# solonas13/REAL

Hardware: NVIDIA B200
Metric: matching-path reads/s (higher is better)
Workload: dtype u64

## Files before the change

### real_b200/csrc/index.cuh

```cuda
#pragma once

#include "common.cuh"
#include "prims.cuh"

namespace realgpu
{

__host__ __device__ __forceinline__ int list_of(int table, int t)
{
        return table == 0 ? (t == 0 ? 0 : (t == 1 ? 3 : 5)) : (table == 1 ? (t == 0 ? 1 : 4) : 2);
}
__host__ __device__ __forceinline__ int pair_second(int table, int t) { return t + 1 + table; }

__host__ __device__ __forceinline__ int table_lists(int table, uint32_t seedkmax)
{
        if ( seedkmax >= 2 ) return table == 0 ? 3 : (table == 1 ? 2 : 1);
        if ( seedkmax == 1 ) return table == 0 ? 2 : (table == 1 ? 1 : 0);
        return table == 0 ? 1 : 0;
}


__device__ __forceinline__ uint64_t pack_bytes(const uint8_t * __restrict__ p, uint32_t len, uint32_t & bad)
{
        uintptr_t const addr = reinterpret_cast<uintptr_t>(p);
// ... 661 lines not shown
                #pragma unroll
                for ( int k = 0; k < 4; ++k )
                        if ( i0 + (uint32_t)k * 256 < s1 )
                        {
                                uint32_t const l = entry_slot(seed[k], G, val[k] & 3) - slot0;
                                atomicOr(&bits[l >> 5], 1u << (l & 31));
                        }
        }
        __syncthreads();
        uint32_t const wpt = (words + 255) / 256;
        uint32_t const w0 = threadIdx.x * wpt;
        uint32_t c = 0;
        for ( uint32_t w = w0; w < min(words, w0 + wpt); ++w ) c += __popc(bits[w]);
        uint32_t d;
        uint32_t run = s0 + block_excl_scan(c, &d);
        for ( uint32_t w = w0; w < min(words, w0 + wpt); ++w ) { rank[w] = run; run += __popc(bits[w]); }
        __syncthreads();
        for ( uint32_t w = threadIdx.x; w < words; w += 256 )
        {
                SlotWord sw; sw.bits = bits[w]; sw.rank = rank[w];
                slots[(uint64_t)sb * words + w] = sw;
        }
        for ( uint32_t r = threadIdx.x; r < d; r += 256 ) E[s0 + r].next = ENTRY_NONE;
        if ( threadIdx.x == 0 && d ) atomicAdd(ndistinct, d);
        __syncthreads();
        for ( uint32_t i0 = s0 + threadIdx.x; i0 < s1; i0 += 1024 )
        {
                uint64_t seed[4]; uint32_t val[4];
                #pragma unroll
                for ( int k = 0; k < 4; ++k )
                {
                        uint32_t const i = i0 + (uint32_t)k * 256;
                        seed[k] = (i < s1) ? __ldg(ent_seed + i) : 0;
                        val[k] = (i < s1) ? __ldg(ent_val + i) : 0;
                }
                #pragma unroll
                for ( int k = 0; k < 4; ++k )
                        if ( i0 + (uint32_t)k * 256 < s1 )
                        {
                                uint32_t const l = entry_slot(seed[k], G, val[k] & 3) - slot0;
                                uint32_t const bit = 1u << (l & 31);
                                uint32_t const r = rank[l >> 5] + __popc(bits[l >> 5] & (bit - 1));
                                if ( ! (atomicOr(&claimed[l >> 5], bit) & bit) )
                                {
                                        E[r].seed = seed[k];
                                        E[r].val = val[k];
                                }
                                else
                                {
                                        uint32_t const j = atomicAdd(&ndup, 1u);
                                        if ( j < SUB_DUP_CAP )
                                        {
                                                SubDup dd; dd.seed = seed[k]; dd.val = val[k]; dd.r = r;
                                                dup[j] = dd;
                                        }
                                        else
                                        {
                                                uint32_t const o = s0 + d + SUB_DUP_CAP + atomicAdd(&ovf, 1u);
                                                Entry en; en.seed = seed[k]; en.val = val[k];
                                                en.next = atomicExch(&E[r].next, o);
                                                E[o] = en;
                                        }
                                }
                        }
        }
        __syncthreads();
        uint32_t const nd = min(ndup, SUB_DUP_CAP);
        for ( uint32_t j = threadIdx.x; j < nd; j += 256 )
        {
                SubDup const dd = dup[j];
                uint32_t const o = s0 + d + j;
                Entry en; en.seed = dd.seed; en.val = dd.val;
                en.next = atomicExch(&E[dd.r].next, o);
                E[o] = en;
        }
}

static const uint32_t SUB3_DUP_CAP = 256;
struct Build3Params
{
        const uint64_t * item_seed; const uint32_t * item_val; const uint32_t * sub_start;
        TableGeom G[3];
        uint32_t sub_shift, words, first_sub;
        SlotWord * slots[3]; Entry * E[3];
        uint32_t * ndistinct[3];
};

template<bool FAST>
__device__ __forceinline__ uint32_t sub_local_slot(uint64_t seed, TableGeom const & G, uint32_t t, int tb, uint32_t slot0)
{
        if ( FAST )
                return (uint32_t)(seed >> (16u * (2u - t - (uint32_t)tb))) & 0xFFFFu;
        return entry_slot(seed, G, t) - slot0;
}

#ifndef REAL_BUILD_MINB
#define REAL_BUILD_MINB 6
#endif
template<bool SPLIT, bool FAST>
__global__ void __launch_bounds__(256, SPLIT ? REAL_BUILD_MINB : 3) k_build_sub3(const __grid_constant__ Build3Params P)
{
        extern __shared__ __align__(16) uint32_t sub_smem[];
        uint32_t const words = P.words;
        constexpr int NT = SPLIT ? 1 : 3;
        __shared__ SubDup dup[NT][SUB3_DUP_CAP];
        __shared__ uint32_t ndup[NT], dist[NT];
        uint32_t const sb = P.first_sub + (SPLIT ? blockIdx.x / 3 : blockIdx.x);
        int const tb0 = SPLIT ? (int)(blockIdx.x % 3) : 0;
        if ( SPLIT && ! P.G[tb0].nlists ) return;
        uint32_t const s0 = P.sub_start[sb], s1 = P.sub_start[sb+1];
        uint32_t const slot0 = sb << P.sub_shift;
        uint32_t const tstride = 2 * words + (words + 1) / 2;
        for ( uint32_t i = s0 + threadIdx.x * 16; i < s1; i += 256 * 16 )
        {
                asm volatile("prefetch.global.L2 [%0];" :: "l"(P.item_seed + i));
                if ( ((i - s0) & 31) == 0 ) asm volatile("prefetch.global.L2 [%0];" :: "l"(P.item_val + i));
        }
        for ( uint32_t w = threadIdx.x; w < NT * tstride; w += 256 ) sub_smem[w] = 0;
        if ( threadIdx.x < NT ) ndup[threadIdx.x] = 0;
        __syncthreads();
        for ( uint32_t i0 = s0 + threadIdx.x; i0 < s1; i0 += 1024 )
        {
                uint64_t seed[4]; uint32_t val[4];
                #pragma unroll
                for ( int k = 0; k < 4; ++k )
                {
                        uint32_t const i = i0 + (uint32_t)k * 256;
                        seed[k] = (i < s1) ? __ldg(P.item_seed + i) : 0;
                        val[k] = (i < s1) ? __ldg(P.item_val + i) : 0;
                }
                #pragma unroll
                for ( int k = 0; k < 4; ++k )
                        if ( i0 + (uint32_t)k * 256 < s1 )
                        {
                                uint32_t const t = val[k] & 3;
                                #pragma unroll
                                for ( int u = 0; u < NT; ++u )
                                {
                                        int const tb = tb0 + u;
                                        if ( t < P.G[tb].nlists )
                                        {
                                                uint32_t const l = sub_local_slot<FAST>(seed[k], P.G[tb], t, tb, slot0);
                                                atomicOr(&sub_smem[u * tstride + (l >> 5)], 1u << (l & 31));
                                        }
                                }
                        }
        }
        __syncthreads();
        uint32_t const wpt = (words + 255) / 256;
        uint32_t const w0 = threadIdx.x * wpt;
        #pragma unroll 1
        for ( int u = 0; u < NT; ++u )
        {
                uint32_t * bits = sub_smem + u * tstride;
                uint16_t * rank = reinterpret_cast<uint16_t *>(bits + 2 * words);
                uint32_t c = 0;
                for ( uint32_t w = w0; w < min(words, w0 + wpt); ++w ) c += __popc(bits[w]);
                uint32_t d;
                uint32_t run = block_excl_scan(c, &d);
                for ( uint32_t w = w0; w < min(words, w0 + wpt); ++w ) { rank[w] = (uint16_t)run; run += __popc(bits[w]); }
                if ( threadIdx.x == 0 ) dist[u] = d;
        }
        __syncthreads();
        #pragma unroll 1
        for ( int u = 0; u < NT; ++u )
        {
// ... 2 lines not shown
                const uint32_t * bits = sub_smem + u * tstride;
                const uint16_t * rank = reinterpret_cast<const uint16_t *>(bits + 2 * words);
                for ( uint32_t w = threadIdx.x; w < words; w += 256 )
                {
                        SlotWord sw; sw.bits = bits[w]; sw.rank = s0 + rank[w];
                        P.slots[tb][(uint64_t)sb * words + w] = sw;
                }
                if ( threadIdx.x == 0 && dist[u] ) atomicAdd(P.ndistinct[tb], dist[u]);
        }
        __syncthreads();
        for ( uint32_t i0 = s0 + threadIdx.x; i0 < s1; i0 += 1024 )
        {
                uint64_t seed[4]; uint32_t val[4];
                #pragma unroll
                for ( int k = 0; k < 4; ++k )
                {
                        uint32_t const i = i0 + (uint32_t)k * 256;
                        seed[k] = (i < s1) ? __ldg(P.item_seed + i) : 0;
                        val[k] = (i < s1) ? __ldg(P.item_val + i) : 0;
                }
                #pragma unroll
                for ( int k = 0; k < 4; ++k )
                        if ( i0 + (uint32_t)k * 256 < s1 )
                        {
                                uint32_t const t = val[k] & 3;
                                #pragma unroll
                                for ( int u = 0; u < NT; ++u )
                                {
                                        int const tb = tb0 + u;
                                        if ( t < P.G[tb].nlists )
                                        {
                                                uint32_t * bits = sub_smem + u * tstride, * claimed = bits + words;
                                                const uint16_t * rank = reinterpret_cast<const uint16_t *>(bits + 2 * words);
                                                uint32_t const l = sub_local_slot<FAST>(seed[k], P.G[tb], t, tb, slot0);
                                                uint32_t const bit = 1u << (l & 31);
                                                uint32_t const r = s0 + rank[l >> 5] + __popc(bits[l >> 5] & (bit - 1));
                                                Entry * E = P.E[tb];
                                                if ( ! (atomicOr(&claimed[l >> 5], bit) & bit) )
                                                {
                                                        Entry en; en.seed = seed[k]; en.val = val[k]; en.next = ENTRY_NONE;
                                                        *reinterpret_cast<uint4 *>(E + r) = *reinterpret_cast<const uint4 *>(&en);
                                                }
                                                else
                                                {
                                                        uint32_t const j = atomicAdd(&ndup[u], 1u);
                                                        if ( j < SUB3_DUP_CAP )
                                                        {
                                                                SubDup dd; dd.seed = seed[k]; dd.val = val[k]; dd.r = r;
                                                                dup[u][j] = dd;
                                                        }
                                                        else
                                                        {
                                                                Entry en; en.seed = seed[k]; en.val = val[k]; en.next = r;
                                                                *reinterpret_cast<uint4 *>(E + s0 + dist[u] + j) = *reinterpret_cast<const uint4 *>(&en);
                                                        }
                                                }
                                        }
                                }
                        }
        }
        __syncthreads();
        #pragma unroll 1
        for ( int u = 0; u < NT; ++u )
        {
                uint32_t const nd = min(ndup[u], SUB3_DUP_CAP);
                Entry * E = P.E[tb0 + u];
                for ( uint32_t j = threadIdx.x; j < nd; j += 256 )
                {
                        SubDup const dd = dup[u][j];
                        uint32_t const o = s0 + dist[u] + j;
                        Entry en; en.seed = dd.seed; en.val = dd.val;
                        en.next = atomicExch(&E[dd.r].next, o);
                        *reinterpret_cast<uint4 *>(E + o) = *reinterpret_cast<const uint4 *>(&en);
                }
                for ( uint32_t j = SUB3_DUP_CAP + threadIdx.x; j < ndup[u]; j += 256 )
                {
                        uint32_t const o = s0 + dist[u] + j;
                        uint32_t const r = E[o].next;
                        E[o].next = atomicExch(&E[r].next, o);
                }
        }
}

}
```

### real_b200/csrc/prims.cuh

```cuda
#pragma once

#include "common.cuh"

namespace realgpu
{


static const int SCAN_THREADS = 256;
static const int SCAN_ITEMS = 8;
static const int SCAN_TILE = SCAN_THREADS * SCAN_ITEMS;

__device__ __forceinline__ uint32_t warp_incl_scan(uint32_t v, int lane)
{
        #pragma unroll
        for ( int o = 1; o < 32; o <<= 1 )
        {
                uint32_t const t = __shfl_up_sync(0xffffffffu, v, o);
                if ( lane >= o ) v += t;
        }
        return v;
}

__device__ __forceinline__ void ballot_bit(uint32_t v, uint32_t mask, uint32_t & bal, uint32_t & flip)
{
        asm volatile("{\n\t"
                     ".reg .pred p;\n\t"
                     ".reg .b32 t;\n\t"
                     "and.b32 t, %2, %3;\n\t"
                     "setp.ne.u32 p, t, 0;\n\t"
                     "vote.sync.ballot.b32 %0, p, 0xffffffff;\n\t"
                     "selp.b32 %1, 0, 0xffffffff, p;\n\t"
                     "}" : "=r"(bal), "=r"(flip) : "r"(v), "r"(mask));
}

__device__ __forceinline__ uint32_t peers_u8(uint32_t v, bool ok)
{
        uint32_t peers = __ballot_sync(0xffffffffu, ok);
        #pragma unroll
        for ( int b = 0; b < 8; ++b )
        {
                uint32_t bal, flip;
                ballot_bit(v, 1u << b, bal, flip);
                peers &= bal ^ flip;
        }
        return peers;
}

__device__ __forceinline__ uint32_t peers_low(uint32_t v, bool ok, uint32_t nbits)
{
        uint32_t peers = __ballot_sync(0xffffffffu, ok);
        #pragma unroll
        for ( int b = 0; b < 8; ++b )
                if ( (uint32_t)b < nbits )
                {
                        uint32_t bal, flip;
                        ballot_bit(v, 1u << b, bal, flip);
                        peers &= bal ^ flip;
                }
        return peers;
}

__device__ __forceinline__ uint32_t block_excl_scan(uint32_t v, uint32_t * total)
{
        __shared__ uint32_t warp_sums[32];
        int const lane = threadIdx.x & 31, wid = threadIdx.x >> 5;
        uint32_t const incl = warp_incl_scan(v, lane);
        if ( lane == 31 ) warp_sums[wid] = incl;
        __syncthreads();
        if ( wid == 0 )
        {
                uint32_t s = (lane < (int)(blockDim.x >> 5)) ? warp_sums[lane] : 0;
                s = warp_incl_scan(s, lane);
                warp_sums[lane] = s;
        }
        __syncthreads();
        uint32_t const base = wid ? warp_sums[wid-1] : 0;
        *total = warp_sums[(blockDim.x >> 5) - 1];
        __syncthreads();
        return base + incl - v;
}

__device__ __forceinline__ uint32_t block_excl_scan256(uint32_t v, uint32_t * total, uint32_t * scratch)
{
        int const lane = threadIdx.x & 31, wid = threadIdx.x >> 5;
        uint32_t const incl = warp_incl_scan(v, lane);
        if ( lane == 31 ) scratch[wid] = incl;
        __syncthreads();
        uint32_t base = 0, all = 0;
        #pragma unroll
        for ( int w = 0; w < 8; ++w )
        {
                uint32_t const x = scratch[w];
                if ( w < wid ) base += x;
// ... 80 lines not shown
```

### real_b200/csrc/real_gpu.cu

```cuda
#include "../../include/real_gpu.h"

#include "common.cuh"
#include "prims.cuh"
#include "index.cuh"
#include "scan.cuh"
#include "post.cuh"
#include "ingest.cuh"
#include "format.cuh"

#include <algorithm>
#include <atomic>
#include <chrono>
#include <thread>
#include <cstring>
#include <cstdlib>
#include <cfloat>
#include <vector>
#include <functional>

using namespace realgpu;

namespace
{

// ... 518 lines not shown
                k_ent_scatter_own<<<(unsigned)std::min<uint64_t>(otiles, (uint64_t)h->sm_count * std::max(1, occ_o)), 256, osmem, h->st>>>(EP);
        }
        else
                k_ent_scatter<<<(unsigned)std::min<uint64_t>(etiles, (uint64_t)h->sm_count * std::max(1, occ)), 256, esmem, h->st>>>(EP);
        RG_KERNEL_CHECK();
        launch_count(h, 2);

        const uint64_t * fin_seed = EP.ent_seed; const uint32_t * fin_val = EP.ent_val; const uint32_t * fin_start = EP.bucket_start;
        if ( TP.e2 )
        {
                RG_CUDA(cudaMemsetAsync(EP.sub_count, 0, (size_t)3 * 65600 * 4, h->st));
                k_ent2_hist<<<(unsigned)(h->sm_count * std::max(1, occh)), 256, 0, h->st>>>(EP);
                RG_KERNEL_CHECK(); launch_count(h);
                uint32_t nl = 0;
                exclusive_scan_u32(EP.sub_count, EP.sub_start, (uint64_t)TP.nsub + 1, ptr<uint32_t>(h->ws_stmp), h->st, &nl);
                launch_count(h, nl);
                k_ent2_scatter<<<(unsigned)(h->sm_count * std::max(1, occ2)), 256, esmem, h->st>>>(EP);
                RG_KERNEL_CHECK(); launch_count(h);
                fin_seed = EP.ent2_seed; fin_val = EP.ent2_val; fin_start = EP.sub_start;
        }
        Grouped G; G.seed = fin_seed; G.val = fin_val; G.start = fin_start;
        return G;
}

void build_table(real_gpu * h, int t, TablePlan const & TP)
{
        if ( TP.empty ) return;
        Table & T = h->tab[t];
        EntryPartParams const & EP = TP.EP;
        Grouped const GR = partition_entries(h, TP);
        const uint64_t * fin_seed = GR.seed; const uint32_t * fin_val = GR.val; const uint32_t * fin_start = GR.start;
        k_build_sub<<<TP.own_subs, 256, (size_t)3 * TP.words * 4, h->st>>>(fin_seed, fin_val, fin_start, EP.G, TP.sub_shift, TP.words, ptr<SlotWord>(T.bitmap), ptr<Entry>(T.E), TP.d_ndist, TP.first_sub);
        RG_KERNEL_CHECK(); launch_count(h);
        RG_CUDA(cudaMemcpyAsync(&h->table_counts[2*t], TP.d_total, 8, cudaMemcpyDeviceToHost, h->st));
}

bool build_tables_fused(real_gpu * h, TablePlan * plan)
{
        uint32_t const hb = h->tab[0].hb, fb = 2 * h->F;
        if ( hb != h->keybits || h->nreads == 0 || plan[0].empty ) return false;
        if ( getenv("REAL_GPU_NO_FUSED_BUILD") ) return false;
        uint32_t const nlA = table_lists(0, h->prm.seedkmax);
        uint64_t const cap_items = h->nreads * 2 * nlA;
        uint32_t const pbmin = hb > 16 ? hb - 16 : 0, pbmax = std::min<uint32_t>(std::min<uint32_t>(16, hb > 5 ? hb - 5 : 0), fb);
        if ( pbmin > pbmax ) return false;
        uint32_t pb = 0;
        while ( (cap_items >> pb) > SUB_TARGET_ENTRIES ) ++pb;
        pb = std::min(std::max(pb, pbmin), pbmax);
        if ( h->comm.nranks > 1 && pb < 8 ) return false;

        TablePlan TP = plan[0];
        uint32_t * meta = TP.EP.bucket_count;
        uint32_t const e1 = std::min<uint32_t>(8, pb);
        TP.e2 = pb - e1; TP.nsub = 1u << pb; TP.sub_shift = hb - pb;
        TP.words = TP.sub_shift >= 5 ? (1u << (TP.sub_shift - 5)) : 1u;
        TP.EP.G.table = TABLE_ITEMS; TP.EP.G.nlists = nlA;
        TP.EP.ebits = e1; TP.EP.e2bits = TP.e2;
        TP.first_sub = 0; TP.own_subs = TP.nsub;
        if ( h->comm.nranks > 1 )
        {
                TP.first_sub = TP.EP.own_lo << (pb - 8);
                TP.own_subs = (TP.EP.own_last + 1 - TP.EP.own_lo) << (pb - 8);
        }
        Build3Params B;
        memset(&B, 0, sizeof(B));
        for ( int t = 0; t < 3; ++t )
        {
                Table & T = h->tab[t];
                T.nblocks = TP.nsub;
                T.bitmap_bytes = (size_t)TP.nsub * TP.words * sizeof(SlotWord);
                dev_reserve(h, T.bitmap, T.bitmap_bytes);
                dev_reserve(h, T.E, std::max<size_t>(16, cap_items * sizeof(Entry)) + 256);
                if ( plan[t].empty ) RG_CUDA(cudaMemsetAsync(T.bitmap.p, 0, T.bitmap_bytes, h->st));
                B.G[t] = plan[t].EP.G; B.G[t].table = t; B.G[t].nlists = plan[t].empty ? 0 : T.nlists;
                B.slots[t] = ptr<SlotWord>(T.bitmap); B.E[t] = ptr<Entry>(T.E);
                B.ndistinct[t] = meta + 521 + t;
        }
        EntryPartParams3 Q;
        for ( int t = 0; t < 3; ++t ) { Q.P[t] = TP.EP; if ( t ) Q.P[t].G.nlists = 0; }
        k_ent_hist3<<<(unsigned)(h->sm_count * 8), 256, 0, h->st>>>(Q);
        RG_KERNEL_CHECK(); launch_count(h);
        Grouped const GR = partition_entries(h, TP);
        B.item_seed = GR.seed; B.item_val = GR.val; B.sub_start = GR.start;
        B.sub_shift = TP.sub_shift; B.words = TP.words; B.first_sub = TP.first_sub;
        bool split = true;
        if ( const char * e = getenv("REAL_GPU_BUILD_SPLIT") ) split = atoi(e) != 0;
        size_t const smem1 = (size_t)(2 * TP.words + (TP.words + 1) / 2) * 4;
        size_t const smem = split ? smem1 : 3 * smem1;
        bool const fast = h->F == 8 && hb == 32 && TP.sub_shift == 16 && ! getenv("REAL_GPU_BUILD_GENERAL");
        typedef void (*build_fn)(const Build3Params);
        build_fn const kb = split ? (fast ? (build_fn)k_build_sub3<true, true> : (build_fn)k_build_sub3<true, false>)
                                  : (fast ? (build_fn)k_build_sub3<false, true> : (build_fn)k_build_sub3<false, false>);
        RG_CUDA(cudaFuncSetAttribute(kb, cudaFuncAttributeMaxDynamicSharedMemorySize, (int)smem));
        kb<<<split ? TP.own_subs * 3 : TP.own_subs, 256, smem, h->st>>>(B);
        RG_KERNEL_CHECK(); launch_count(h);
        RG_CUDA(cudaMemcpyAsync(&h->table_counts[0], TP.d_total, 16, cudaMemcpyDeviceToHost, h->st));
        h->fused_build = true;
        return true;
}

int build_from_device(real_gpu * h)
{
        uint32_t const seedl = std::min<uint32_t>(h->prm.seedl, 32);
        h->F = seedl / 4;
        h->keybits = seedl;
        h->W = std::max<uint32_t>(1, (h->maxlen + 31) / 32);
        uint64_t const nreads = h->nreads;

        RG_CUDA(cudaEventRecord(h->ev[2], h->st));
        if ( ! h->src_packed )
                dev_reserve(h, h->rpack, (size_t)nreads * 2 * h->W * 8 + 16);
        dev_reserve(h, h->rlen, (size_t)nreads * 4 + 16);
        dev_reserve(h, h->seeds, (size_t)nreads * 2 * 8 + 16);
        dev_reserve(h, h->usable, (size_t)nreads * 4 + 16);
        dev_reserve(h, h->bad, (size_t)nreads * 4 + 16);
        if ( ! h->src_packed && h->W > PB_MAX_W )
                RG_CUDA(cudaMemsetAsync(h->bad.p, 0, (size_t)nreads * 4 + 16, h->st));
        if ( nreads )
        {
                if ( ! h->src_packed && h->W <= PB_MAX_W )
                {
                        uint32_t const rpb = 256 / h->W;
                        k_pack_both<<<blocks_for(nreads, rpb), 256, 0, h->st>>>(h->src_mapped, ptr<uint64_t>(h->offs), nreads, h->W, seedl, h->prm.seedl, ptr<uint64_t>(h->rpack),
                                                                                ptr<uint32_t>(h->rlen), ptr<uint64_t>(h->seeds), ptr<uint32_t>(h->usable));
                        RG_KERNEL_CHECK(); launch_count(h);
                }
                else if ( h->src_packed )
                {
                        k_seeds_packed<<<blocks_for(nreads, 256), 256, 0, h->st>>>(h->src_packed, h->src_byte_offsets,
                                                                                 (h->src_packed_uniform || h->src_len32) ? nullptr : ptr<uint64_t>(h->offs), h->src_len32,
                                                                                 h->src_packed_uniform, nreads, seedl, h->prm.seedl, ptr<uint32_t>(h->bad),
                                                                                 ptr<uint32_t>(h->rlen), ptr<uint64_t>(h->seeds), ptr<uint32_t>(h->usable));
                        RG_KERNEL_CHECK(); launch_count(h);
                }
                else
                {
                        k_pack_reads<<<blocks_for(nreads * 2 * h->W, 256), 256, 0, h->st>>>(h->src_mapped, ptr<uint64_t>(h->offs), nreads, h->W,
                                                                                          ptr<uint64_t>(h->rpack), ptr<uint32_t>(h->bad));
                        RG_KERNEL_CHECK(); launch_count(h);
                        k_read_seeds<<<blocks_for(nreads, 256), 256, 0, h->st>>>(ptr<uint64_t>(h->offs), nreads, h->W, seedl, h->prm.seedl, ptr<uint64_t>(h->rpack),
                                                                               ptr<uint32_t>(h->bad), ptr<uint32_t>(h->rlen), ptr<uint64_t>(h->seeds), ptr<uint32_t>(h->usable));
                        RG_KERNEL_CHECK(); launch_count(h);
                }
        }
        RG_CUDA(cudaEventRecord(h->ev[3], h->st));

        uint64_t const maxent = std::max<uint64_t>(1, nreads * 2 * table_lists(0, h->prm.seedkmax));
        uint32_t const hbmax = std::min<uint32_t>(h->keybits, 32);
        dev_reserve(h, h->ws_k0, maxent * 8 + 16);
        dev_reserve(h, h->ws_v0, maxent * 4 + 16);
        dev_reserve(h, h->ws_k1, maxent * 8 + 16);
        dev_reserve(h, h->ws_v1, maxent * 4 + 16);
        dev_reserve(h, h->ws_flags, (size_t)3 * 65600 * 4);
        dev_reserve(h, h->ws_stmp, scan_temp_elems(65600) * 4 + 64);
        dev_reserve(h, h->ws_hist, 3 * TABLE_META_WORDS * 4);
        memset(h->table_counts, 0, 6 * sizeof(uint32_t));
        TablePlan plan[3];
        EntryPartParams3 Q;
        bool any_table = false;
        for ( int t = 0; t < 3; ++t )
        {
                plan[t] = plan_table(h, t, ptr<uint32_t>(h->ws_hist) + (size_t)t * TABLE_META_WORDS);
                Q.P[t] = plan[t].EP;
                any_table = any_table || ! plan[t].empty;
        }
        h->fused_build = false;
        if ( any_table && build_tables_fused(h, plan) )
                any_table = false;
        else
        for ( int t = 0; t < 3 && any_table; ++t )
                if ( ! plan[t].empty )
                {
// ... 458 lines not shown
                        if ( sharded )
                        {
                                comm_signal(h, 0);
                                comm_wait(h, 0, CM.epoch, S.wait_ms);
                                k_comm_pairs<<<1, SC_PAIR_THREADS, 0, h->st>>>(P, reinterpret_cast<uint32_t *>(CM.base[CM.rank] + CM.meta_off));
                                RG_KERNEL_CHECK(); launch_count(h);
                        }
                        mark();
                        if ( h->evp.size() < 2 * (nprobe_ev + 1) )
                        {
                                cudaEvent_t a, b;
                                RG_CUDA(cudaEventCreate(&a)); RG_CUDA(cudaEventCreate(&b));
                                h->evp.push_back(a); h->evp.push_back(b);
                        }
                        if ( h->text_pending ) RG_CUDA(cudaStreamWaitEvent(h->st, h->evc[1], 0));
                        RG_CUDA(cudaEventRecord(h->evp[2 * nprobe_ev], h->st));
                        S.probe<<<(unsigned)(h->sm_count * S.occ_b), SC_THREADS, S.bsmem, h->st>>>(P);
                        RG_KERNEL_CHECK();
                        RG_CUDA(cudaEventRecord(h->evp[2 * nprobe_ev + 1], h->st));
                        ++nprobe_ev;
                        mark();
                        if ( sharded )
                        {
                                comm_signal(h, 1);
                        }
                        launch_count(h);
                        h->stats.scan_launches += 1;
                }
                P.x_begin = x_begin; P.x_end = x_end;
                RG_CUDA(cudaMemcpyAsync(ptr<unsigned long long>(h->counters) + 4, P.nprobed, 8, cudaMemcpyDeviceToDevice, h->st));
                if ( ! sharded && x_end - x_begin <= chunk_cap )
                {
                        R.x_begin = S.x_begin; R.x_end = S.x_end; R.win_begin = P.win_begin; R.win_end = P.win_end; R.chunk_cap = S.chunk_cap;
                        R.bucket_bits = P.bucket_bits; R.own_b_lo = P.own_b_lo; R.own_b_cnt = P.own_b_cnt; R.own_list = S.own_list; R.recs = P.recs;
                        R.valid = true; R.ahead = false;
                }
                if ( trace )
                {
                        RG_CUDA(cudaStreamSynchronize(h->st));
                        static const char * names[6] = { "hist", "wait_consumed", "offsets+scatter", "handover", "probe", "" };
                        for ( size_t i = 0; i + 1 < tev.size(); ++i )
                        {
                                if ( i % 6 == 5 ) continue;
                                fprintf(stderr, "[trace rank %u round %zu] %-16s %8.3f ms\n", CM.rank, i / 6, names[i % 6], elapsed(tev[i], tev[i+1]));
                        }
                        for ( cudaEvent_t e : tev ) cudaEventDestroy(e);
                }
        }
        RG_CUDA(cudaEventRecord(h->ev[6], h->st));
        unsigned long long c[5] = {0, 0, 0, 0, 0};
        RG_CUDA(cudaMemcpyAsync(c, h->counters.p, sizeof(c), cudaMemcpyDeviceToHost, h->st));
        RG_CUDA(cudaStreamSynchronize(h->st));
        R.inflight = false;
        h->stats.scan_ms = elapsed(h->ev[5], h->ev[6]);
        finish_text(h);
        h->stats.probe_ms = 0;
        for ( size_t i = 0; i < nprobe_ev; ++i ) h->stats.probe_ms += elapsed(h->evp[2*i], h->evp[2*i+1]);
        h->stats.part_ms = was_ahead ? elapsed(R.ev0, R.done) : (use_prep ? 0.f : h->stats.scan_ms - h->stats.probe_ms);
        h->stats.prepared_scans += was_ahead ? 1 : 0;
        if ( ! ntiles ) h->stats.n_windows = 0;
        else if ( h->comm.nranks > 1 && ! h->comm.window.p ) h->stats.n_windows = c[4];
        if ( h->comm.nranks > 1 && h->comm.window.p )
        {
                uint32_t cerr = 0;
                RG_CUDA(cudaMemcpy(&cerr, h->comm.error.p, 4, cudaMemcpyDeviceToHost));
                if ( cerr ) throw CudaError("sharded tables: timed out waiting for rank " + std::to_string(cerr - 1));
        }
        uint32_t nt = 0;
        for ( int t = 0; t < 3; ++t ) if ( P.tab[t].nlists ) ++nt;
        h->stats.n_probes = h->stats.n_windows * nt;
        h->stats.n_candidates = c[1];
        h->stats.n_seedpass = c[2];
        h->stats.n_hits = c[3];
        return (mode != 1) ? (uint64_t)c[0] : (uint64_t)c[3];
}

void preload_kernels(int device)
{
        static bool done[64] = { false };
        if ( device < 0 || device >= 64 || done[device] ) return;
        cudaFuncAttributes a;
#define RG_PRELOAD(k) RG_CUDA(cudaFuncGetAttributes(&a, k))
        RG_PRELOAD(k_pack_reads); RG_PRELOAD(k_pack_both); RG_PRELOAD(k_seeds_packed); RG_PRELOAD(k_read_seeds); RG_PRELOAD(k_uniform_offsets); RG_PRELOAD(k_flags_to_bad);
        RG_PRELOAD(k_ent_hist3); RG_PRELOAD(k_ent_offsets); RG_PRELOAD(k_ent_scatter); RG_PRELOAD(k_ent_scatter_own); RG_PRELOAD(k_ent2_hist); RG_PRELOAD(k_ent2_scatter); RG_PRELOAD(k_build_sub); RG_PRELOAD((k_build_sub3<true, true>)); RG_PRELOAD((k_build_sub3<true, false>)); RG_PRELOAD((k_build_sub3<false, true>)); RG_PRELOAD((k_build_sub3<false, false>));
        RG_PRELOAD(k_scan_reduce); RG_PRELOAD(k_scan_apply); RG_PRELOAD(k_fill_f32);
        RG_PRELOAD(k_part_hist); RG_PRELOAD(k_part_offsets); RG_PRELOAD(k_part_scatter<false>); RG_PRELOAD(k_part_scatter<true>); RG_PRELOAD(k_own_list); RG_PRELOAD((k_bucket_probe<false, false>)); RG_PRELOAD((k_bucket_probe<true, false>)); RG_PRELOAD((k_bucket_probe<false, true>)); RG_PRELOAD((k_bucket_probe<true, true>));
        RG_PRELOAD(k_comm_signal); RG_PRELOAD(k_comm_wait); RG_PRELOAD(k_comm_pairs);
        RG_PRELOAD(k_score_hits); RG_PRELOAD(k_hit_count); RG_PRELOAD(k_hit_scatter); RG_PRELOAD(k_hit_order<real_gpu_hit>);
        RG_PRELOAD(k_unique_export); RG_PRELOAD(k_unique_ties); RG_PRELOAD(k_unique_import); RG_PRELOAD(k_unique_replay); RG_PRELOAD(k_fold_push); RG_PRELOAD(k_fold_merge); RG_PRELOAD(k_unique_checksum); RG_PRELOAD(k_mark_large); RG_PRELOAD(k_sort_large<0>); RG_PRELOAD(k_sort_large<1>); RG_PRELOAD(k_sort_large<2>);
        RG_PRELOAD(k_fmt_len<false>); RG_PRELOAD(k_fmt_len<true>); RG_PRELOAD(k_fmt_write<false>); RG_PRELOAD(k_fmt_write<true>);
        RG_PRELOAD(k_fa_summary); RG_PRELOAD(k_rd_table); RG_PRELOAD(k_rd_permute); RG_PRELOAD(k_rd_repack); RG_PRELOAD(k_rd_sums); RG_PRELOAD(k_fa_scan); RG_PRELOAD(k_fa_pack);
        RG_PRELOAD(k_window_counts); RG_PRELOAD(k_block_bounds); RG_PRELOAD(k_gap_dp); RG_PRELOAD(k_gap_replay);
#undef RG_PRELOAD
        done[device] = true;
}

int check_ready(real_gpu * h)
{
        if ( ! h->have_text ) return fail(h, REAL_GPU_E_STATE, "no text set");
        if ( ! h->have_reads ) return fail(h, REAL_GPU_E_STATE, "no reads set");
        if ( std::min<uint64_t>(h->n_total, h->own_end + h->maxlen) > h->shard_begin + h->shard_len )
                return fail(h, REAL_GPU_E_ARG, "the shard does not hold the read-length halo behind its own range (real_gpu_set_text: [own_begin, min(n_total, own_end + maxreadlen)))");
        return REAL_GPU_OK;
}

}


extern "C" {

int real_gpu_abi_version(void) { return REAL_GPU_ABI_VERSION; }

int real_gpu_device_count(void)
{
        int n = 0;
        if ( cudaGetDeviceCount(&n) != cudaSuccess ) { (void)cudaGetLastError(); return 0; }
        return n;
}

int real_gpu_create(const real_gpu_params * params, real_gpu ** out)
{
        if ( ! params || ! out ) return REAL_GPU_E_ARG;
        *out = nullptr;
        if ( params->struct_size != sizeof(real_gpu_params) ) return REAL_GPU_E_ARG;
        real_gpu * h = new real_gpu();
        h->prm = *params;
        h->prm.ll_table = nullptr;
        int code = REAL_GPU_OK;
        try
        {
                if ( params->seedl < 4 || params->seedl > 64 || params->seedl % 4 )
                        throw std::invalid_argument("seed length must be a multiple of 4 in 4..64");
                if ( params->seedkmax > 2 ) throw std::invalid_argument("seedkmax > 2");
                if ( params->totalkmax > 15 ) throw std::invalid_argument("totalkmax > 15");
                if ( params->scores && ! params->ll_table ) throw std::invalid_argument("scores requested without ll_table");
                int ndev = 0;
                RG_CUDA(cudaGetDeviceCount(&ndev));
                if ( params->device < 0 || params->device >= ndev ) throw CudaError("no such CUDA device");
                RG_CUDA(cudaSetDevice(params->device));
                cudaDeviceProp prop;
                RG_CUDA(cudaGetDeviceProperties(&prop, params->device));
                if ( prop.major < 10 ) throw CudaError("device is not sm_100 class; this library only carries sm_100a code");
                h->sm_count = prop.multiProcessorCount;
                preload_kernels(params->device);
                if ( const char * e = getenv("REAL_GPU_PASS_BITS") ) h->pass_bits_override = atoi(e);
                if ( const char * e = getenv("REAL_GPU_L2_SLICE_MB") ) h->l2_slice_bytes = (uint64_t)atoi(e) << 20;
                if ( const char * e = getenv("REAL_GPU_OWN_LIST_MAX") ) h->own_list_max = atoi(e);
                if ( const char * e = getenv("REAL_GPU_AUTO_PREPARE") ) h->auto_prepare = atoi(e) != 0;
                if ( const char * e = getenv("REAL_GPU_CHUNK_MPOS") ) h->chunk_positions = std::max<uint64_t>(SC_TILE_POS, ((uint64_t)atoi(e) << 20) / SC_TILE_POS * SC_TILE_POS);
                RG_CUDA(cudaStreamCreateWithFlags(&h->st, cudaStreamNonBlocking));
                RG_CUDA(cudaStreamCreateWithFlags(&h->st2, cudaStreamNonBlocking));
                RG_CUDA(cudaMallocHost(&h->table_counts, 6 * sizeof(uint32_t)));
                RG_CUDA(cudaMallocHost(&h->fa_totals, 2 * sizeof(uint64_t)));
                for ( int i = 0; i < 8; ++i ) RG_CUDA(cudaEventCreate(&h->ev[i]));
                for ( int i = 0; i < 2; ++i ) RG_CUDA(cudaEventCreate(&h->evc[i]));
                RG_CUDA(cudaEventCreateWithFlags(&h->ev_words, cudaEventDisableTiming));
                if ( params->ll_table )
                {
                        dev_alloc(h, h->ll, 1024 * 8);
                        RG_CUDA(cudaMemcpyAsync(h->ll.p, params->ll_table, 1024 * 8, cudaMemcpyHostToDevice, h->st));
                        RG_CUDA(cudaStreamSynchronize(h->st));
                }
        }
        catch ( std::invalid_argument const & e ) { h->err = e.what(); code = REAL_GPU_E_ARG; }
        catch ( std::exception const & e ) { h->err = e.what(); code = REAL_GPU_E_CUDA; }
        if ( code != REAL_GPU_OK )
        {
// ... 1422 lines not shown
```

### real_b200/csrc/scan.cuh

```cuda
#pragma once

#include "common.cuh"
#include "index.cuh"

namespace realgpu
{

static const int SC_THREADS = 256;
static const int SC_WPT = 2;
static const int SC_TILE_WORDS = SC_THREADS * SC_WPT;
static const int SC_TILE_POS = SC_TILE_WORDS * 32;
static const int SC_HALO = 2;
static const int SC_SMEM_WORDS = SC_TILE_WORDS + 2 * SC_HALO;
static const int SC_MAX_BUCKETS = 256;
static const int SC_CURSOR_STRIDE = 32;
static const int SC_UNIT = 512;
#ifndef REAL_SC_RPT
#define REAL_SC_RPT 2
#endif
#ifndef REAL_PROBE_MINB
#define REAL_PROBE_MINB 3
#endif
static const int SC_RPT = REAL_SC_RPT;
static const int SC_QA_CAP = 32 + 96 * SC_RPT;
static const int SC_QB_CAP = 64;
static const uint32_t SC_POS_NONE = 0xFFFFFFFFu;
static const uint64_t SC_MAX_CHUNK = 0xFFF00000ull;
static const uint64_t SC_MAX_ROUND = 1ull << 30;

static const int SC_MAX_RANKS = 8;
static const int SC_META_STRIDE = SC_MAX_BUCKETS + 8;

struct TableDev
{
        const SlotWord * slots;
        const Entry * E;
        uint32_t hb;
        uint32_t nlists;
};

struct ScanParams
{
        const uint64_t * text;
        const uint64_t * nmask;
        uint64_t shard_begin;
        uint64_t x_begin, x_end;
        uint64_t pos_base;
        uint64_t win_begin, win_end;
        uint64_t own_begin, own_end;
        TableDev tab[3];
        uint32_t seedl, F, keybits, seedkmax, totalkmax;
        uint32_t vseedl;
        ReadSrc rs;
        const uint32_t * rlen;
        const uint64_t * rec;
        uint32_t nrec;
        uint32_t fileid;
        uint32_t bucket_bits;
        uint32_t debug_flags;
        uint4 * recs;
        uint32_t * bucket_count;
        uint32_t * bucket_start;
        uint32_t * bucket_cursor;
        uint32_t * unit_counter;
        int mode;
        RawHit * hits;
        unsigned long long hit_cap;
        unsigned long long * hit_count;
        unsigned long long * info;
        unsigned long long * stats;
        uint32_t nranks, rank;
        uint32_t bucket_lo[SC_MAX_RANKS + 1];
        uint4 * peer_recs[SC_MAX_RANKS];
        uint32_t * peer_meta[SC_MAX_RANKS];
        uint32_t seg_cap;
        uint32_t * pair_grab;
        uint32_t * pair_rec;
        uint32_t npairs;
        uint32_t own_b_lo, own_b_cnt;
        uint32_t hist_pick_max;
        uint32_t * list;
        unsigned long long * list_count;
        unsigned long long * nprobed;
};

__device__ __forceinline__ uint32_t bucket_owner(ScanParams const & P, uint32_t b)
{
        uint32_t r = 0;
        #pragma unroll
        for ( int i = 1; i < SC_MAX_RANKS; ++i )
                if ( (uint32_t)i < P.nranks && b >= P.bucket_lo[i] ) r = i;
        return r;
}

__device__ __forceinline__ uint32_t smem_u32(const void * p) { return (uint32_t)__cvta_generic_to_shared(p); }

__device__ __forceinline__ void mbar_init(uint64_t * bar, uint32_t count)
{
        asm volatile("mbarrier.init.shared::cta.b64 [%0], %1;" :: "r"(smem_u32(bar)), "r"(count));
}
__device__ __forceinline__ void mbar_expect_tx(uint64_t * bar, uint32_t bytes)
{
        asm volatile("mbarrier.arrive.expect_tx.shared::cta.b64 _, [%0], %1;" :: "r"(smem_u32(bar)), "r"(bytes) : "memory");
}
__device__ __forceinline__ void mbar_wait(uint64_t * bar, uint32_t parity)
{
        uint32_t done = 0;
        while ( ! done )
        {
                asm volatile(
                        "{\n\t"
                        ".reg .pred p;\n\t"
                        "mbarrier.try_wait.parity.shared::cta.b64 p, [%1], %2;\n\t"
                        "selp.u32 %0, 1, 0, p;\n\t"
                        "}" : "=r"(done) : "r"(smem_u32(bar)), "r"(parity) : "memory");
        }
}
__device__ __forceinline__ void bulk_load(void * dst, const void * src, uint32_t bytes, uint64_t * bar)
{
        asm volatile("cp.async.bulk.shared::cluster.global.mbarrier::complete_tx::bytes [%0], [%1], %2, [%3];"
                     :: "r"(smem_u32(dst)), "l"(src), "r"(bytes), "r"(smem_u32(bar)) : "memory");
}


__device__ __forceinline__ void unique_update(unsigned long long * slot, uint32_t inverted, uint32_t file, uint64_t pos, uint32_t k, uint32_t frag)
{
        unsigned long long old = *slot;
        while ( true )
        {
                uint32_t const st = umi_state(old);
                unsigned long long const take = umi_make(inverted ? ST_REVERSE : ST_STRAIGHT, file, pos, k, frag);
                unsigned long long neu = old;
                if ( st == ST_NOMATCH || st == ST_GAPPED )
                        neu = take;
                else if ( k < umi_err(old) )
                        neu = take;
                else if ( k == umi_err(old) )
                {
                        bool const same = (pos == umi_pos(old)) && (file == umi_file(old)) && (frag == umi_frag(old));
                        if ( st == ST_NONUNIQUE )
                        {
                                if ( file < umi_file(old) || (file == umi_file(old) && pos < umi_pos(old)) )
                                        neu = umi_with_state(take, ST_NONUNIQUE);
                        }
                        else if ( ! same )
                        {
                                bool const smaller = file < umi_file(old) || (file == umi_file(old) && pos < umi_pos(old));
                                neu = umi_with_state(smaller ? take : old, ST_NONUNIQUE);
                        }
                        else if ( ! inverted && st == ST_REVERSE )
                                neu = take;
                }
                if ( neu == old )
                        return;
                unsigned long long const prev = atomicCAS(slot, old, neu);
                if ( prev == old )
                        return;
                old = prev;
        }
}

__device__ __forceinline__ uint32_t record_of(const uint64_t * __restrict__ rec, uint32_t nrec, uint64_t pos)
{
        uint32_t lo = 0, hi = nrec + 1;
        while ( lo < hi )
        {
                uint32_t const mid = (lo + hi) >> 1;
                if ( __ldg(rec + mid) <= pos ) lo = mid + 1; else hi = mid;
        }
        return lo - 1;
}

__device__ __forceinline__ bool wildcard_free(const uint64_t * __restrict__ nmask, uint64_t lpos, uint32_t len)
{
        uint64_t const first = lpos >> 6, last = (lpos + len - 1) >> 6;
        for ( uint64_t w = first; w <= last; ++w )
        {
                uint64_t m = __ldg(nmask + w);
                if ( m )
                {
                        if ( w == first ) m &= (~0ULL) >> (lpos & 63);
                        if ( w == last ) m &= (~0ULL) << (63 - ((lpos + len - 1) & 63));
                        if ( m ) return false;
                }
        }
        return true;
}



struct HistSmem
{
        uint64_t tile[2][SC_SMEM_WORDS];
        uint64_t bar[2];
        uint32_t cnt[SC_MAX_BUCKETS];
};

__device__ __forceinline__ uint32_t clip_mask(uint64_t lx0, uint64_t x_begin, uint64_t x_end)
{
        if ( lx0 + 32 <= x_begin || lx0 >= x_end ) return 0;
        uint32_t m = 0xFFFFFFFFu;
        if ( lx0 < x_begin ) m &= 0xFFFFFFFFu << (uint32_t)(x_begin - lx0);
        if ( lx0 + 32 > x_end ) m &= 0xFFFFFFFFu >> (uint32_t)(lx0 + 32 - x_end);
        return m;
}

// ... 880 lines not shown
```

Baseline: 579.1 million.

## Add persistent fused 3-table sub-bucket build kernel with bulk-copy double buffering

Adds a persistent kernel that loops over sub-buckets, building all three tables in shared memory per sub-bucket. While one sub-bucket is processed, the next one's seeds and values are prefetched with cp.async.bulk into a second buffer tracked by an mbarrier. The aim is to hide global load latency and avoid per-sub-bucket launch and block scheduling overhead. It uses large shared memory at one block per SM with 1024 threads, which may cut latency hiding elsewhere. Sub-buckets too large for the buffer fall back to reading directly from global memory.

```diff
diff --git a/real_b200/csrc/index.cuh b/real_b200/csrc/index.cuh
--- a/real_b200/csrc/index.cuh
+++ b/real_b200/csrc/index.cuh
@@ -767,6 +767,7 @@
         const uint64_t * item_seed; const uint32_t * item_val; const uint32_t * sub_start;
         TableGeom G[3];
         uint32_t sub_shift, words, first_sub;
+        uint32_t nsubs;
         SlotWord * slots[3]; Entry * E[3];
         uint32_t * ndistinct[3];
 };
@@ -935,4 +936,207 @@
         }
 }
 
-}
+static const uint32_t B3_WORDS = 2048;
+static const uint32_t B3_TSTRIDE = 2 * B3_WORDS + B3_WORDS / 2;
+static const uint32_t B3_ITEM_CAP = 6400;
+template<uint32_t NTHR>
+struct Build3Smem
+{
+        uint64_t seed[2][B3_ITEM_CAP + 2];
+        uint32_t val[2][B3_ITEM_CAP + 8];
+        uint32_t tab[3][B3_TSTRIDE];
+        SubDup dup[3][SUB3_DUP_CAP];
+        uint64_t wsum[NTHR / 32];
+        uint64_t bar[2];
+        uint32_t ndup[3], dist[3];
+};
+
+__device__ __forceinline__ bool b3_fits(uint32_t s0, uint32_t s1) { return s1 > s0 && s1 - s0 <= B3_ITEM_CAP; }
+
+template<uint32_t NTHR>
+__device__ __forceinline__ void b3_fetch(Build3Smem<NTHR> & S, Build3Params const & P, uint32_t buf, uint32_t s0, uint32_t s1)
+{
+        uint32_t const a = s0 & ~1u, b = (s1 + 1) & ~1u, c = s0 & ~3u, d = (s1 + 3) & ~3u;
+        mbar_expect_tx(&S.bar[buf], (b - a) * 8 + (d - c) * 4);
+        bulk_load(S.seed[buf], P.item_seed + a, (b - a) * 8, &S.bar[buf]);
+        bulk_load(S.val[buf], P.item_val + c, (d - c) * 4, &S.bar[buf]);
+}
+
+template<uint32_t NTHR>
+__device__ __forceinline__ void b3_clear(Build3Smem<NTHR> & S)
+{
+        #pragma unroll
+        for ( int tb = 0; tb < 3; ++tb )
+                for ( uint32_t w = threadIdx.x; w < 2 * B3_WORDS / 4; w += NTHR )
+                        reinterpret_cast<uint4 *>(S.tab[tb])[w] = make_uint4(0u, 0u, 0u, 0u);
+}
+
+template<uint32_t NTHR>
+__device__ __forceinline__ void b3_build(Build3Smem<NTHR> & S, Build3Params const & P, uint32_t sb, uint32_t s0, uint32_t n,
+                                         const uint64_t * isd, const uint32_t * ivl)
+{
+        constexpr uint32_t WPT = B3_WORDS / NTHR;
+        static_assert(WPT % 2 == 0, "slot words are stored two at a time");
+        for ( uint32_t i = threadIdx.x; i < n; i += NTHR )
+        {
+                uint64_t const seed = isd[i];
+                uint32_t const t = ivl[i] & 3;
+                #pragma unroll
+                for ( int tb = 0; tb < 3; ++tb )
+                        if ( t < P.G[tb].nlists )
+                        {
+                                uint32_t const l = sub_local_slot<true>(seed, P.G[tb], t, tb, 0);
+                                atomicOr(&S.tab[tb][l >> 5], 1u << (l & 31));
+                        }
+        }
+        __syncthreads();
+        uint32_t const w0 = threadIdx.x * WPT;
+        uint32_t bw[3][WPT];
+        uint64_t cnt = 0;
+        #pragma unroll
+        for ( int tb = 0; tb < 3; ++tb )
+        {
+                uint32_t c = 0;
+                #pragma unroll
+                for ( uint32_t k = 0; k < WPT; ++k ) { bw[tb][k] = S.tab[tb][w0 + k]; c += __popc(bw[tb][k]); }
+                cnt |= (uint64_t)c << (21 * tb);
+        }
+        int const lane = threadIdx.x & 31, wid = threadIdx.x >> 5;
+        uint64_t incl = cnt;
+        #pragma unroll
+        for ( int o = 1; o < 32; o <<= 1 )
+        {
+                uint64_t const x = __shfl_up_sync(0xffffffffu, incl, o);
+                if ( lane >= o ) incl += x;
+        }
+        if ( lane == 31 ) S.wsum[wid] = incl;
+        __syncthreads();
+        uint64_t base = 0, all = 0;
+        #pragma unroll
+        for ( int w = 0; w < (int)(NTHR / 32); ++w )
+        {
+                uint64_t const x = S.wsum[w];
+                if ( w < wid ) base += x;
+                all += x;
+        }
+        uint64_t const ex = base + incl - cnt;
+        #pragma unroll
+        for ( int tb = 0; tb < 3; ++tb )
+        {
+                uint16_t * rank = reinterpret_cast<uint16_t *>(S.tab[tb] + 2 * B3_WORDS);
+                uint32_t run = (uint32_t)(ex >> (21 * tb)) & 0x1FFFFFu;
+                uint32_t rk[WPT];
+                #pragma unroll
+                for ( uint32_t k = 0; k < WPT; ++k ) { rk[k] = run; rank[w0 + k] = (uint16_t)run; run += __popc(bw[tb][k]); }
+                if ( P.G[tb].nlists )
+                {
+                        uint4 * dst = reinterpret_cast<uint4 *>(P.slots[tb] + (uint64_t)sb * B3_WORDS + w0);
+                        #pragma unroll
+                        for ( uint32_t k = 0; k < WPT; k += 2 ) dst[k / 2] = make_uint4(bw[tb][k], s0 + rk[k], bw[tb][k+1], s0 + rk[k+1]);
+                }
+        }
+        if ( threadIdx.x < 3 )
+        {
+                uint32_t const d = (uint32_t)(all >> (21 * threadIdx.x)) & 0x1FFFFFu;
+                S.dist[threadIdx.x] = d;
+                S.ndup[threadIdx.x] = 0;
+                if ( P.G[threadIdx.x].nlists && d ) atomicAdd(P.ndistinct[threadIdx.x], d);
+        }
+        __syncthreads();
+        for ( uint32_t i = threadIdx.x; i < n; i += NTHR )
+        {
+                uint64_t const seed = isd[i];
+                uint32_t const val = ivl[i], t = val & 3;
+                #pragma unroll
+                for ( int tb = 0; tb < 3; ++tb )
+                        if ( t < P.G[tb].nlists )
+                        {
+                                uint32_t * bits = S.tab[tb], * claimed = bits + B3_WORDS;
+                                const uint16_t * rank = reinterpret_cast<const uint16_t *>(bits + 2 * B3_WORDS);
+                                uint32_t const l = sub_local_slot<true>(seed, P.G[tb], t, tb, 0);
+                                uint32_t const bit = 1u << (l & 31);
+                                uint32_t const r = s0 + rank[l >> 5] + __popc(bits[l >> 5] & (bit - 1));
+                                Entry * E = P.E[tb];
+                                if ( ! (atomicOr(&claimed[l >> 5], bit) & bit) )
+                                {
+                                        Entry en; en.seed = seed; en.val = val; en.next = ENTRY_NONE;
+                                        *reinterpret_cast<uint4 *>(E + r) = *reinterpret_cast<const uint4 *>(&en);
+                                }
+                                else
+                                {
+                                        uint32_t const j = atomicAdd(&S.ndup[tb], 1u);
+                                        if ( j < SUB3_DUP_CAP )
+                                        {
+                                                SubDup dd; dd.seed = seed; dd.val = val; dd.r = r;
+                                                S.dup[tb][j] = dd;
+                                        }
+                                        else
+                                        {
+                                                Entry en; en.seed = seed; en.val = val; en.next = r;
+                                                *reinterpret_cast<uint4 *>(E + s0 + S.dist[tb] + j) = *reinterpret_cast<const uint4 *>(&en);
+                                        }
+                                }
+                        }
+        }
+        __syncthreads();
+        #pragma unroll 1
+        for ( int tb = 0; tb < 3; ++tb )
+        {
+                uint32_t const nd = min(S.ndup[tb], SUB3_DUP_CAP);
+                Entry * E = P.E[tb];
+                for ( uint32_t j = threadIdx.x; j < nd; j += NTHR )
+                {
+                        SubDup const dd = S.dup[tb][j];
+                        uint32_t const o = s0 + S.dist[tb] + j;
+                        Entry en; en.seed = dd.seed; en.val = dd.val;
+                        en.next = atomicExch(&E[dd.r].next, o);
+                        *reinterpret_cast<uint4 *>(E + o) = *reinterpret_cast<const uint4 *>(&en);
+                }
+                for ( uint32_t j = SUB3_DUP_CAP + threadIdx.x; j < S.ndup[tb]; j += NTHR )
+                {
+                        uint32_t const o = s0 + S.dist[tb] + j;
+                        uint32_t const r = E[o].next;
+                        E[o].next = atomicExch(&E[r].next, o);
+                }
+        }
+        b3_clear(S);
+        __syncthreads();
+}
+
+template<uint32_t NTHR>
+__global__ void __launch_bounds__(NTHR, 1) k_build_sub3_persist(const __grid_constant__ Build3Params P)
+{
+        extern __shared__ __align__(16) unsigned char b3_smem[];
+        Build3Smem<NTHR> & S = *reinterpret_cast<Build3Smem<NTHR> *>(b3_smem);
+        if ( threadIdx.x == 0 )
+        {
+                mbar_init(&S.bar[0], 1);
+                mbar_init(&S.bar[1], 1);
+                asm volatile("fence.mbarrier_init.release.cluster;" ::: "memory");
+        }
+        b3_clear(S);
+        __syncthreads();
+        const uint32_t * start = P.sub_start + P.first_sub;
+        if ( threadIdx.x == 0 && blockIdx.x < P.nsubs && b3_fits(start[blockIdx.x], start[blockIdx.x + 1]) )
+                b3_fetch(S, P, 0, start[blockIdx.x], start[blockIdx.x + 1]);
+        uint32_t phase = 0;
+        uint32_t it = 0;
+        for ( uint32_t sb = blockIdx.x; sb < P.nsubs; sb += gridDim.x, ++it )
+        {
+                uint32_t const buf = it & 1;
+                uint32_t const s0 = start[sb], s1 = start[sb + 1];
+                uint32_t const nb = sb + gridDim.x;
+                if ( threadIdx.x == 0 && nb < P.nsubs && b3_fits(start[nb], start[nb + 1]) )
+                        b3_fetch(S, P, buf ^ 1, start[nb], start[nb + 1]);
+                if ( b3_fits(s0, s1) )
+                {
+                        mbar_wait(&S.bar[buf], (phase >> buf) & 1);
+                        phase ^= 1u << buf;
+                        b3_build(S, P, P.first_sub + sb, s0, s1 - s0, S.seed[buf] + (s0 & 1), S.val[buf] + (s0 & 3));
+                }
+                else
+                        b3_build(S, P, P.first_sub + sb, s0, s1 - s0, P.item_seed + s0, P.item_val + s0);
+        }
+}
+
+}
diff --git a/real_b200/csrc/prims.cuh b/real_b200/csrc/prims.cuh
--- a/real_b200/csrc/prims.cuh
+++ b/real_b200/csrc/prims.cuh
@@ -9,6 +9,35 @@
 static const int SCAN_THREADS = 256;
 static const int SCAN_ITEMS = 8;
 static const int SCAN_TILE = SCAN_THREADS * SCAN_ITEMS;
+
+__device__ __forceinline__ uint32_t smem_u32(const void * p) { return (uint32_t)__cvta_generic_to_shared(p); }
+
+__device__ __forceinline__ void mbar_init(uint64_t * bar, uint32_t count)
+{
+        asm volatile("mbarrier.init.shared::cta.b64 [%0], %1;" :: "r"(smem_u32(bar)), "r"(count));
+}
+__device__ __forceinline__ void mbar_expect_tx(uint64_t * bar, uint32_t bytes)
+{
+        asm volatile("mbarrier.arrive.expect_tx.shared::cta.b64 _, [%0], %1;" :: "r"(smem_u32(bar)), "r"(bytes) : "memory");
+}
+__device__ __forceinline__ void mbar_wait(uint64_t * bar, uint32_t parity)
+{
+        uint32_t done = 0;
+        while ( ! done )
+        {
+                asm volatile(
+                        "{\n\t"
+                        ".reg .pred p;\n\t"
+                        "mbarrier.try_wait.parity.shared::cta.b64 p, [%1], %2;\n\t"
+                        "selp.u32 %0, 1, 0, p;\n\t"
+                        "}" : "=r"(done) : "r"(smem_u32(bar)), "r"(parity) : "memory");
+        }
+}
+__device__ __forceinline__ void bulk_load(void * dst, const void * src, uint32_t bytes, uint64_t * bar)
+{
+        asm volatile("cp.async.bulk.shared::cluster.global.mbarrier::complete_tx::bytes [%0], [%1], %2, [%3];"
+                     :: "r"(smem_u32(dst)), "l"(src), "r"(bytes), "r"(smem_u32(bar)) : "memory");
+}
 
 __device__ __forceinline__ uint32_t warp_incl_scan(uint32_t v, int lane)
 {
diff --git a/real_b200/csrc/real_gpu.cu b/real_b200/csrc/real_gpu.cu
--- a/real_b200/csrc/real_gpu.cu
+++ b/real_b200/csrc/real_gpu.cu
@@ -624,12 +624,29 @@
         RG_KERNEL_CHECK(); launch_count(h);
         Grouped const GR = partition_entries(h, TP);
         B.item_seed = GR.seed; B.item_val = GR.val; B.sub_start = GR.start;
-        B.sub_shift = TP.sub_shift; B.words = TP.words; B.first_sub = TP.first_sub;
+        B.sub_shift = TP.sub_shift; B.words = TP.words; B.first_sub = TP.first_sub; B.nsubs = TP.own_subs;
         bool split = true;
         if ( const char * e = getenv("REAL_GPU_BUILD_SPLIT") ) split = atoi(e) != 0;
         size_t const smem1 = (size_t)(2 * TP.words + (TP.words + 1) / 2) * 4;
         size_t const smem = split ? smem1 : 3 * smem1;
         bool const fast = h->F == 8 && hb == 32 && TP.sub_shift == 16 && ! getenv("REAL_GPU_BUILD_GENERAL");
+        bool persistent = fast && split && TP.words == B3_WORDS;
+        if ( const char * e = getenv("REAL_GPU_BUILD_PERSISTENT") ) persistent = persistent && atoi(e) != 0;
+        if ( persistent )
+        {
+                unsigned const nthr = getenv("B3_THR512") ? 512 : 1024;
+                typedef void (*build_fn)(const Build3Params);
+                build_fn const kp = nthr == 512 ? (build_fn)k_build_sub3_persist<512> : (build_fn)k_build_sub3_persist<1024>;
+                size_t const psmem = nthr == 512 ? sizeof(Build3Smem<512>) : sizeof(Build3Smem<1024>);
+                RG_CUDA(cudaFuncSetAttribute(kp, cudaFuncAttributeMaxDynamicSharedMemorySize, (int)psmem));
+                int occ = 0;
+                RG_CUDA(cudaOccupancyMaxActiveBlocksPerMultiprocessor(&occ, kp, nthr, psmem));
+                kp<<<(unsigned)std::min<uint64_t>(TP.own_subs, (uint64_t)h->sm_count * std::max(1, occ)), nthr, psmem, h->st>>>(B);
+                RG_KERNEL_CHECK(); launch_count(h);
+                RG_CUDA(cudaMemcpyAsync(&h->table_counts[0], TP.d_total, 16, cudaMemcpyDeviceToHost, h->st));
+                h->fused_build = true;
+                return true;
+        }
         typedef void (*build_fn)(const Build3Params);
         build_fn const kb = split ? (fast ? (build_fn)k_build_sub3<true, true> : (build_fn)k_build_sub3<true, false>)
                                   : (fast ? (build_fn)k_build_sub3<false, true> : (build_fn)k_build_sub3<false, false>);
@@ -1254,7 +1271,7 @@
         cudaFuncAttributes a;
 #define RG_PRELOAD(k) RG_CUDA(cudaFuncGetAttributes(&a, k))
         RG_PRELOAD(k_pack_reads); RG_PRELOAD(k_pack_both); RG_PRELOAD(k_seeds_packed); RG_PRELOAD(k_read_seeds); RG_PRELOAD(k_uniform_offsets); RG_PRELOAD(k_flags_to_bad);
-        RG_PRELOAD(k_ent_hist3); RG_PRELOAD(k_ent_offsets); RG_PRELOAD(k_ent_scatter); RG_PRELOAD(k_ent_scatter_own); RG_PRELOAD(k_ent2_hist); RG_PRELOAD(k_ent2_scatter); RG_PRELOAD(k_build_sub); RG_PRELOAD((k_build_sub3<true, true>)); RG_PRELOAD((k_build_sub3<true, false>)); RG_PRELOAD((k_build_sub3<false, true>)); RG_PRELOAD((k_build_sub3<false, false>));
+        RG_PRELOAD(k_ent_hist3); RG_PRELOAD(k_ent_offsets); RG_PRELOAD(k_ent_scatter); RG_PRELOAD(k_ent_scatter_own); RG_PRELOAD(k_ent2_hist); RG_PRELOAD(k_ent2_scatter); RG_PRELOAD(k_build_sub); RG_PRELOAD((k_build_sub3<true, true>)); RG_PRELOAD((k_build_sub3<true, false>)); RG_PRELOAD((k_build_sub3<false, true>)); RG_PRELOAD((k_build_sub3<false, false>)); RG_PRELOAD(k_build_sub3_persist<1024>); RG_PRELOAD(k_build_sub3_persist<512>);
         RG_PRELOAD(k_scan_reduce); RG_PRELOAD(k_scan_apply); RG_PRELOAD(k_fill_f32);
         RG_PRELOAD(k_part_hist); RG_PRELOAD(k_part_offsets); RG_PRELOAD(k_part_scatter<false>); RG_PRELOAD(k_part_scatter<true>); RG_PRELOAD(k_own_list); RG_PRELOAD((k_bucket_probe<false, false>)); RG_PRELOAD((k_bucket_probe<true, false>)); RG_PRELOAD((k_bucket_probe<false, true>)); RG_PRELOAD((k_bucket_probe<true, true>));
         RG_PRELOAD(k_comm_signal); RG_PRELOAD(k_comm_wait); RG_PRELOAD(k_comm_pairs);
diff --git a/real_b200/csrc/scan.cuh b/real_b200/csrc/scan.cuh
--- a/real_b200/csrc/scan.cuh
+++ b/real_b200/csrc/scan.cuh
@@ -93,35 +93,6 @@
         return r;
 }
 
-__device__ __forceinline__ uint32_t smem_u32(const void * p) { return (uint32_t)__cvta_generic_to_shared(p); }
-
-__device__ __forceinline__ void mbar_init(uint64_t * bar, uint32_t count)
-{
-        asm volatile("mbarrier.init.shared::cta.b64 [%0], %1;" :: "r"(smem_u32(bar)), "r"(count));
-}
-__device__ __forceinline__ void mbar_expect_tx(uint64_t * bar, uint32_t bytes)
-{
-        asm volatile("mbarrier.arrive.expect_tx.shared::cta.b64 _, [%0], %1;" :: "r"(smem_u32(bar)), "r"(bytes) : "memory");
-}
-__device__ __forceinline__ void mbar_wait(uint64_t * bar, uint32_t parity)
-{
-        uint32_t done = 0;
-        while ( ! done )
-        {
-                asm volatile(
-                        "{\n\t"
-                        ".reg .pred p;\n\t"
-                        "mbarrier.try_wait.parity.shared::cta.b64 p, [%1], %2;\n\t"
-                        "selp.u32 %0, 1, 0, p;\n\t"
-                        "}" : "=r"(done) : "r"(smem_u32(bar)), "r"(parity) : "memory");
-        }
-}
-__device__ __forceinline__ void bulk_load(void * dst, const void * src, uint32_t bytes, uint64_t * bar)
-{
-        asm volatile("cp.async.bulk.shared::cluster.global.mbarrier::complete_tx::bytes [%0], [%1], %2, [%3];"
-                     :: "r"(smem_u32(dst)), "l"(src), "r"(bytes), "r"(smem_u32(bar)) : "memory");
-}
-
 
 __device__ __forceinline__ void unique_update(unsigned long long * slot, uint32_t inverted, uint32_t file, uint64_t pos, uint32_t k, uint32_t frag)
 {
```

Measured after the change: 568.5 million (median of 6 runs). 1.8% lower.
